# UMEssen/Body-and-Organ-Analysis

Measured on AMD Instinct MI355X. Metric: CT volumes/sec (512^3 @1.5 mm, total+bca) on MI355X, higher is better.
Workload: dtype f16

## Files before the change

body-and-organ-analysis_amd/boa_hip/_lib.py:

```python
from __future__ import annotations

import ctypes as C
import os

_HERE = os.path.dirname(os.path.abspath(__file__))
LIB_PATH = os.environ.get("BOA_HIP_LIB") or os.path.join(_HERE, "libboa_hip.so")

BOA_OK, BOA_EINVAL, BOA_EHIP, BOA_ENOMEM, BOA_EINF = 0, -1, -2, -3, -4
K_CONV_MFMA, K_CONV_FIRST, K_CONVT, K_NORM_FINALIZE, K_HEAD_ACCUM, K_ARGMAX, K_OTHER, K_AGG, K_MORPH, K_RESAMPLE, K_COPY, K_COUNT = range(12)
K_NAMES = ["conv_mfma", "conv_first", "convT_mfma", "norm_finalize", "head_accum", "finalize_argmax", "other", "aggregation",
           "morphology", "resample", "copy_remap"]
CNT_NAMES = ["head_mfma", "head_valu", "conv_ws", "conv_simple", "first_mfma", "first_valu", "f32", "conv_x3", "x3", "head_gather"]
MAX_STAGES = 8


class NetDesc(C.Structure):
    _fields_ = [
        ("n_stages", C.c_int), ("in_channels", C.c_int), ("num_classes", C.c_int),
        ("features", C.c_int * MAX_STAGES), ("kernel", (C.c_int * 3) * MAX_STAGES),
        ("stride", (C.c_int * 3) * MAX_STAGES), ("n_conv_enc", C.c_int * MAX_STAGES),
        ("n_conv_dec", C.c_int * MAX_STAGES), ("patch", C.c_int * 3), ("norm_eps", C.c_float),
        ("lrelu_slope", C.c_float),
    ]

# ... 39 lines not shown
    "boa_finalize_labels": (i32, [vp, vp, vp, i32, ip, vp, i32, i32, i32, vp, i32, vp, ip, ip, vp]),
    "boa_finalize_labels_planes": (i32, [vp, vp, vp, i32, ip, vp, i32, i32, i32, vp, i32, vp, ip, ip, vp, i32, i32]),
    "boa_net_predict_sliding_window_deferred": (i32, [vp, vp, ip, ip, ip, ip, i32, vp, vp, vp, ip, C.POINTER(vp)]),
    "boa_net_apply_deferred": (i32, [vp, vp, vp, vp, vp, ip]),
    "boa_stash_destroy": (None, [vp]),
    "boa_net_create": (i32, [vp, C.POINTER(NetDesc), vp, u64, i32, i32, C.POINTER(vp)]),
    "boa_net_destroy": (None, [vp]),
    "boa_net_weight_count": (u64, [C.POINTER(NetDesc)]),
    "boa_net_load_weights": (i32, [vp, vp, u64]),
    "boa_net_set_mirroring": (i32, [vp, i32]),
    "boa_net_forward": (i32, [vp, vp, ip, ip, i32, vp]),
    "boa_net_predict_sliding_window": (i32, [vp, vp, ip, ip, ip, ip, i32, vp, vp, vp]),
    "boa_net_labels_supported": (i32, [vp, ip, i32]),
    "boa_net_predict_labels_fold": (i32, [vp, vp, ip, ip, ip, ip, i32, vp, vp, i32, i32, vp, i32, vp, ip, ip, vp]),
    "boa_conv_block_test": (i32, [vp, vp, i32, i32, ip, vp, vp, vp, vp, i32, ip, ip, i32, i32, vp]),
    "boa_convtranspose_test": (i32, [vp, vp, i32, i32, ip, vp, vp, i32, ip, vp]),
    "boa_tissue_aggregate": (i32, [vp, vp, vp, vp, vp, vp, i32, i32, i32, vp, vp]),
    "boa_slice_label_presence": (i32, [vp, vp, i32, i32, i32, vp]),
    "boa_tissue_projections": (i32, [vp, vp, vp, i32, i32, i32, vp, i32, vp, vp, vp, vp]),
    "boa_label_hu_histogram": (i32, [vp, vp, vp, vp, u64, i32, i32, vp]),
    "boa_label_hu_mask": (i32, [vp, vp, vp, vp, i32, i32, i32, u64, vp]),
    "boa_group_stats_f64": (i32, [vp, vp, vp, u64, vp, i32, vp, vp]),
    "boa_label_hu_mask_f64": (i32, [vp, vp, vp, vp, i32, C.c_double, C.c_double, u64, vp]),
    "boa_tissue_aggregate_f64": (i32, [vp, vp, vp, vp, vp, vp, i32, i32, i32, vp, vp]),
    "boa_binary_erode": (i32, [vp, vp, vp, vp, i32, i32, i32, i32]),
    "boa_ccl26": (i32, [vp, vp, i32, i32, i32, vp, vp, ip]),
    "boa_ccl_filter_largest": (i32, [vp, vp, vp, u64, vp, i32]),
    "boa_ccl_remove_small": (i32, [vp, vp, vp, u64, C.c_uint32, vp]),
    "boa_ccl_list_components": (i32, [vp, vp, u64, i32, vp, vp, ip]),
    "boa_scatter_u32": (i32, [vp, vp, vp, vp, i32]),
# ... 78 lines not shown
```

body-and-organ-analysis_amd/csrc/conv.h:

```cpp
#pragma once
#include "common.h"

struct ActSrc {
    const __half* data = nullptr;
    const float* ss = nullptr;
    const unsigned* ss16 = nullptr;
    int C = 0;
};

struct ConvGeom {
    int N, Di, Hi, Wi, Do, Ho, Wo;
    int Cout;
    int k[3], s[3];
    int Cin;
};

struct ConvTile {
    int variant;
    int R;
    int w[3];
    int b[3];
    int h[3];
    int xs;
    int tiles[3];
// ... 14 lines not shown
void pack_convt_weights(const float* w , int Cin, int Cout, const int s[3], __half* dst);

int launch_conv_mfma(boa_ctx* ctx, const ActSrc& s0, const ActSrc& s1, const ConvGeom& g, const ConvTile& t,
                     const __half* wpk, const float* bias, float slope, __half* out, float* partials);
int conv_nblk(const ConvTile& t, int cu_count, int Cout);
int conv_ws_nslots(int tiles_per_sample, int cu_count);
int launch_conv_x3(boa_ctx* ctx, const float* src0, const float* ss0, int C0, const float* src1, const float* ss1, int C1,
                   const ConvGeom& g, const ConvTile& t, const __half* wpk, float wscale, const float* bias, float slope, float* out,
                   float* partials);

int launch_norm_finalize(boa_ctx* ctx, float* partials, int nblk, int N, int C, double count,
                         const float* gamma, const float* beta, float eps, float* ss_out, unsigned* ss16_out, int clear);

bool first_mfma_ok(int Cin, const int P[3], const int k[3], int Cout);
bool conv_ws_row_reuse(int R, int k1, int s1, int w1, int b1, int b2);
int convt_mfma_form(int Cin, const int s[3], bool norm_src);
int convt_x3_mt(size_t vin);

int launch_conv_first(boa_ctx* ctx, const float* volume, const int V[3], const int vol_off[3], const int* dev_origins,
                      int N, int Cin, const int P[3], const int k[3], int Cout, const float* w, const float* bias,
                      float* padded_scratch, __half* out, float* partials, int* nblk_out, int flip_mask = 0, float* out32 = nullptr);
int conv_first_nblk(const int P[3], int cu_count);
void conv_first_padded_dims(const int P[3], const int k[3], int out[3]);

int launch_convt_mfma(boa_ctx* ctx, const ActSrc& src, int N, const int din[3], const int s[3], int Cout,
                      const __half* wpk, const float* bias, float slope, __half* out);

int launch_head(boa_ctx* ctx, const __half* act, const float* ss, int F0, const int P[3], int C, const float* w,
                const float* bias, float slope, float* logits_out, const uint16_t* gauss, uint16_t* acc,
                uint16_t* nacc, const int PV[3], const int start[3], size_t plane_stride = 0);
// ... 86 lines not shown
```

body-and-organ-analysis_amd/csrc/conv.hip:

```cpp
#include <stdlib.h>
#include <string.h>

#include <algorithm>
#include <cmath>

#include "conv.h"


size_t conv_wpk_halves(int Cin_total, int Cout, const int k[3]) {
    return (size_t)(Cin_total / 16) * k[0] * k[1] * k[2] * 2 * Cout * 8;
}

void pack_conv_weights(const float* w, int Cin, int Cout, const int k[3], __half* dst) {
    const int taps = k[0] * k[1] * k[2];
    for (int co = 0; co < Cout; ++co)
        for (int ci = 0; ci < Cin; ++ci)
            for (int t = 0; t < taps; ++t) {
                int cc = ci / 16, kh = (ci % 16) / 8, j = ci % 8;
                size_t o = ((((size_t)cc * taps + t) * 2 + kh) * Cout + co) * 8 + j;
                dst[o] = __float2half_rn(w[((size_t)co * Cin + ci) * taps + t]);
            }
}

size_t convt_wpk_halves(int Cin, int Cout, const int s[3]) { return (size_t)s[0] * s[1] * s[2] * Cin * Cout; }
// ... 104 lines not shown
                            if (b0 * b1 * b2 != M) continue;
                            const int b[3] = {b0, b1, b2};
                            int h[3], tl[3];
                            long long HV = 1, covered = 1, tiles = 1;
                            for (int d = 0; d < 3; ++d) {
                                const int ext = b[d] * w[d];
                                h[d] = (ext - 1) * g.s[d] + g.k[d];
                                tl[d] = ceil_div(dims[d], ext);
                                HV *= h[d];
                                covered *= (long long)tl[d] * ext;
                                tiles *= tl[d];
                            }
                            int xs = h[1] * h[2];
                            if (variant == 1 && w0 > 1 && w1 == 1 && w2 >= 8 && w2 <= 16 && g.s[0] == 1 && g.s[2] == 1)
                                while (xs % 16 != w2 % 16) ++xs;
                            if (variant == 1) HV = (long long)h[0] * xs;
                            if (variant == 1 && !conv_ws_supported(g.k, (int)HV)) continue;
                            const size_t lds = variant == 1 ? conv_ws_lds_bytes((int)HV, taps, ncc, g.Cout)
                                                            : conv_lds_bytes((int)HV, taps);
                            if (lds > 160 * 1024 - 2048) continue;
                            const long long nblocks = tiles * (g.Cout / 32) * g.N;
                            const double valid = (double)dims[0] * dims[1] * dims[2];
                            const double waste = (double)covered / valid;
                            const double lds_pen = (g.s[2] > 1 ? 1.25 : 1.0) * (w2 < 16 ? 1.3 : (w2 < 32 ? 1.15 : 1.0));
                            const double t_mfma = (double)taps * R * 32.0 * lds_pen * (x3 ? 2.0 : 1.0);
                            double t_chunk;
                            const double slots = cu_count;
                            if (variant == 1) {
                                const bool res = conv_ws_resident((int)HV, taps, ncc, g.Cout);
                                const double t_prod = (double)h[0] * h[1] * h[2] * 4.3 + (res ? 0.0 : taps * 64.0 / 256.0 * 60.0) + 800.0;
// ... 416 lines not shown
```

body-and-organ-analysis_amd/csrc/conv_ws.hip:

```cpp
#include <stdlib.h>

#include "conv.h"
#include "conv_ws_dev.h"

__global__ __launch_bounds__(64) void k_ws_build_desc(ConvArgs p, int grid, int row, int* __restrict__ out) {
    const int b = (int)blockIdx.x * 64 + (int)threadIdx.x;
    if (b >= grid) return;
    int* r = out + (size_t)b * row * 8;
    int my = 0;
    for (int v = b; v < p.N * p.vw; v += grid) my += p.runs[(v % p.vw) * 8];
    if (my > row - 1) my = row - 1;
    r[0] = my;
    for (int i = 1; i < 8; ++i) r[i] = 0;
    TileSeq s;
    s.n = s.left = s.j = 0;
    for (int k = 0; k < my; ++k) {
        bool new_run = true;
        if (k == 0)
            seq_first_of(p, s, b);
        else
            new_run = seq_next(p, s);
        const TileDesc d = make_desc(p, s, new_run);
        int* e = r + (size_t)(k + 1) * 8;
        e[0] = d.tc.n; e[1] = d.tc.cy; e[2] = d.tc.ox0; e[3] = d.tc.oy0; e[4] = d.tc.oz0; e[5] = d.flags; e[6] = d.vo; e[7] = d.ibase;
// ... 89 lines not shown
            if (jj == 0 || jj == NB - 1)
                __builtin_amdgcn_sched_group_barrier(0x008, 1, 0);
            else if (jj == 1 || jj == NB - 2)
                __builtin_amdgcn_sched_group_barrier(0x008, R >= 2 ? 2 : 1, 0);
            else
                __builtin_amdgcn_sched_group_barrier(0x008, 3, 0);
            (void)cnt;
            if (g + 1 < G) {
                fetch_b(g + 1, jj);
                __builtin_amdgcn_sched_group_barrier(0x100, 1, 0);
            }
        }
    }
}

template <int R, int K0, int K2>
__device__ __forceinline__ void consume_chunk_y_x3(const unsigned char* b0p, const unsigned char* ap, int xs, int h2, int plane, int kh,
                                                   f32x16 (&acc)[R]) {
    constexpr int G = K0 * K2;
    constexpr int NP = G / 2;
    constexpr int NB = R + 2;
    static_assert((G & 1) == 1 && NP >= 1 && R >= 2 && R <= 4, "consume_chunk_y_x3: 3 or 9 groups, 2 .. 4 rows per wave");
    f16x8 ah[2][3], al[2][3];
    f16x8 fh[NB], fl[NB];
    const unsigned char* bhi = b0p - kh * plane;
    auto gtap = [](int g, int dy) { return (((g / K2) * 3 + dy) * K2 + (g % K2)) * 1024; };
    constexpr int GL = G - 1;
    auto fetch_a = [&](int u, int slot) {
        if (u < NP) {
            const int g0 = 2 * u, g1 = g0 + 1;
// ... 89 lines not shown
        for (int r = 0; r < R; ++r) acc[r] = __builtin_amdgcn_mfma_f32_32x32x16_f16(ah[cb][0], fl[r], acc[r], 0, 0, 0);
#pragma unroll
        for (int r = 0; r < R; ++r) acc[r] = __builtin_amdgcn_mfma_f32_32x32x16_f16(al[cb][0], fh[r], acc[r], 0, 0, 0);
#pragma unroll
        for (int r = 0; r < R; ++r) {
            const f16x8& s2 = (r & 1) ? fl[R + r / 2] : fh[R + r / 2];
            acc[r] = __builtin_amdgcn_mfma_f32_32x32x16_f16(ah[cb][2], s2, acc[r], 0, 0, 0);
        }
#pragma unroll
        for (int r = 0; r < R; ++r) {
            const f16x8& s2 = (r & 1) ? fl[R + r / 2] : fh[R + r / 2];
            acc[r] = __builtin_amdgcn_mfma_f32_32x32x16_f16(al[cb][2], s2, acc[r], 0, 0, 0);
        }
    }
}

template <int R, int K0, int K1, int K2, bool YR, bool X3>
__global__ __launch_bounds__(WS_THREADS) void k_conv_ws(ConvArgs p, int total_tiles, int resident_w, int dbg_arg, const int* __restrict__ desc,
                                                        int desc_row) {
#ifdef WS_WITH_TRACE
    const int dbg = dbg_arg;
#else
    constexpr int dbg = 0;
    (void)dbg_arg;
#endif
    extern __shared__ __attribute__((aligned(16))) unsigned char smem[];
    const int tid = threadIdx.x;
    const int lane = tid & 63;
    const int wave = __builtin_amdgcn_readfirstlane(tid >> 6);
    const bool producer = wave >= 4;
    const int l31 = lane & 31;
    const int kh = lane >> 5;
    constexpr int taps = K0 * K1 * K2;
    const int HV = p.h0 * p.xs;
    const int plane = ws_plane_bytes(HV);
    const int ncc = (p.C0 + p.C1) / 16;
    const int wres_bytes = resident_w ? ncc * taps * 1024 : 0;
    const int buf_bytes = resident_w ? 2 * plane : 2 * plane + taps * 1024;
    unsigned char* bufs = smem + wres_bytes;

    const int* __restrict__ drow = desc + (size_t)blockIdx.x * desc_row * 8;
    const int my_tiles = drow[0];
    const int my_chunks = my_tiles * ncc;

    float* const s_bias = (float*)(bufs + 2 * buf_bytes);
    if constexpr (X3) {
        for (int i = tid; i < p.Cout; i += WS_THREADS) s_bias[i] = p.bias[i] * p.wscale;
    }
// ... 75 lines not shown
            if (live && g + 1 < my_chunks) {
                WS_STAMP(1);
                commit(rgA, bufs + ((g + 1) & 1) * buf_bytes);
                if (g + 2 < my_chunks) issue_next(rgA, g + 3 < my_chunks);
                WS_STAMP(3);
            }
            __syncthreads();
        }
        return;
    }

    if (R > 1 && !(dbg & (1024 | 2048))) __builtin_amdgcn_s_setprio(3);
    const int cw = wave & 3;
    int hoff[R];
    {
        const int lz = l31 & (p.w2 - 1);
        const int ly = (l31 >> p.lw2) & (p.w1 - 1);
        const int lx = l31 >> (p.lw2 + p.lw1);
#pragma unroll
        for (int r = 0; r < R; ++r) {
            const int m = cw * R + r;
            const int mz = m & (p.b2 - 1);
            const int my = (m >> p.lb2) & (p.b1 - 1);
            const int mx = m >> (p.lb2 + p.lb1);
            const int tx = mx * p.w0 + lx, ty = my * p.w1 + ly, tz = mz * p.w2 + lz;
            hoff[r] = ((tx * p.s0) * p.xs + (ty * p.s1) * p.h2 + tz * p.s2) * 16 + kh * plane;
        }
    }
    auto vox_rel = [&](int v, int& x, int& y, int& z) {
        x = v >> (p.lw2 + p.lw1);
        y = (v >> p.lw2) & (p.w1 - 1);
        z = v & (p.w2 - 1);
    };
    int srel0;
    {
        int x, y, z;
        vox_rel(l31, x, y, z);
        srel0 = (x * p.Ho + y) * p.Wo + z;
    }
    const size_t out_vox = (size_t)p.Do * p.Ho * p.Wo;
    const int nslots = p.nslots;
    int slot = 0;
    constexpr bool TWO_SETS = (R == 1);
    struct StatSet {
        float s[16], q[16];
    };
    StatSet stA, stB;
#pragma unroll
    for (int i = 0; i < 16; ++i) stA.s[i] = stA.q[i] = stB.s[i] = stB.q[i] = 0.f;
    int st_n = -1, st_cy = 0;
    auto flush_set = [&](StatSet& st, int cy) {
#define WS_HALVE(M, HALF)                                                                                \
    {                                                                                                    \
        const bool up = (l31 & (M)) != 0;                                                                \
        _Pragma("unroll") for (int i = 0; i < (HALF); ++i) {                                             \
            const float ks = up ? st.s[i + (HALF)] : st.s[i], gs = up ? st.s[i] : st.s[i + (HALF)];      \
            const float kq = up ? st.q[i + (HALF)] : st.q[i], gq = up ? st.q[i] : st.q[i + (HALF)];      \
            st.s[i] = ks + __shfl_xor(gs, (M));                                                          \
            st.q[i] = kq + __shfl_xor(gq, (M));                                                          \
        }                                                                                                \
    }
        WS_HALVE(1, 8)
        WS_HALVE(2, 4)
        WS_HALVE(4, 2)
        WS_HALVE(8, 1)
#undef WS_HALVE
        st.s[0] += __shfl_xor(st.s[0], 16);
        st.q[0] += __shfl_xor(st.q[0], 16);
        if (l31 < 16) {
            const int i = ((l31 & 1) << 3) | ((l31 & 2) << 1) | ((l31 & 4) >> 1) | ((l31 & 8) >> 3);
            const int row = cy * 32 + 8 * (i >> 2) + 4 * kh + (i & 3);
            float* pp = p.partials + (((size_t)st_n * p.Cout + row) * 2) * nslots + slot;
            pp[0] = st.s[0];
            pp[nslots] = st.q[0];
        }
#pragma unroll
        for (int i = 0; i < 16; ++i) st.s[i] = st.q[i] = 0.f;
    };
    auto flush_stats = [&]() {
        if (st_n < 0) return;
        if (TWO_SETS && p.cy_fast) {
            flush_set(stA, 0);
            flush_set(stB, 1);
        } else {
            flush_set(stA, st_cy);
        }
    };

    TileDesc cd;
    cd.flags = cd.vo = cd.ibase = 0;
    TileCoord& tc = cd.tc;
    int done_fl = 0, done_vo = 0;
    tc.n = tc.cy = tc.ox0 = tc.oy0 = tc.oz0 = tc.sp = 0;
    if (WS_TRACING && blockIdx.x == 0 && tid == 0) {
        p.trace[WS_TRACE_SLOTS - 4] = __builtin_readcyclecounter();
        p.trace[WS_TRACE_SLOTS - 3] = __builtin_amdgcn_s_memrealtime();
    }
    __syncthreads();
    f32x16 acc[R];
#pragma unroll
    for (int r = 0; r < R; ++r)
#pragma unroll
        for (int i = 0; i < 16; ++i) acc[r][i] = 0.f;
    auto epilogue = [&](const TileCoord& tc, int dfl, int dvo, bool valid) {
        const bool two = TWO_SETS && p.cy_fast;
        if (valid && (tc.n != st_n || (!two && tc.cy != st_cy))) {
            flush_stats();
            st_n = tc.n;
            st_cy = tc.cy;
        }
        const int cout0 = tc.cy * 32;
        const bool full = valid && (dfl & WS_DF_FULL) != 0;
        const size_t ovox = (size_t)(unsigned)dvo;
        const size_t obase = ((size_t)tc.n * p.Cout + cout0) * out_vox + ovox * 16;
        const unsigned olane = ((unsigned)kh * (unsigned)out_vox + (unsigned)srel0) * 32u;
        const unsigned char* const tile_dst = (const unsigned char*)(p.out + obase);
#ifdef WS_TRACE_EPILOGUE
        WS_STAMP(9);
// ... 85 lines not shown
                w[pr * 4 + 2] = cvt_pk_h2(hi4[0], hi4[1]);
                w[pr * 4 + 3] = cvt_pk_h2(hi4[2], hi4[3]);
            }
            if (ok && !(dbg & 4)) {
                WS_GLOBAL unsigned char* dst = sgpr_ptr(tile_dst + (unsigned)mrel * 32u);
                unsigned ol = olane;
                asm volatile("" : "+v"(ol));
                __builtin_nontemporal_store(u32x4_t{w[0], w[1], w[2], w[3]}, (WS_GLOBAL u32x4_t*)(dst + ol));
                __builtin_nontemporal_store(u32x4_t{w[4], w[5], w[6], w[7]}, (WS_GLOBAL u32x4_t*)(dst + ol + 16));
            }
        }
#ifdef WS_TRACE_EPILOGUE
        WS_STAMP(11);
#endif
    };
    f32x16 biasv;
#pragma unroll
    for (int i = 0; i < 16; ++i) biasv[i] = 0.f;
    int bias_cy = -1;
    TileCoord done_tc;
    done_tc.n = done_tc.cy = done_tc.ox0 = done_tc.oy0 = done_tc.oz0 = done_tc.sp = 0;
    for (int k = 0; k < my_tiles + 1; ++k) {
        bool new_run = true;
        const bool more = k < my_tiles;
#ifdef WS_TRACE_EPILOGUE
        WS_STAMP(13);
#endif
        if (more) {
            cd = load_desc(drow, k);
            new_run = (cd.flags & WS_DF_NEWRUN) != 0;
        }
#ifdef WS_TRACE_EPILOGUE
        WS_STAMP(14);
#endif
        if (!(dbg & 8)) epilogue(done_tc, done_fl, done_vo, k > 0);
#pragma unroll
        for (int r = 0; r < R; ++r) asm volatile("" : "=v"(acc[r]));
        if (!more) break;
        if (new_run) {
            flush_stats();
            st_n = -1;
            slot = (int)((unsigned)cd.flags >> 16) * 4 + cw;
        }
        if (!X3 && tc.cy != bias_cy) {
            bias_cy = tc.cy;
            const WS_GLOBAL unsigned char* bbase = sgpr_ptr(p.bias + __builtin_amdgcn_readfirstlane(tc.cy) * 32);
            unsigned bl = (unsigned)kh * 16u;
            asm volatile("" : "+v"(bl));
#pragma unroll
            for (int gq = 0; gq < 4; ++gq) {
                const f32x4_t bv = *(const WS_GLOBAL f32x4_t*)(bbase + bl + 32 * gq);
                biasv[gq * 4 + 0] = bv[0]; biasv[gq * 4 + 1] = bv[1]; biasv[gq * 4 + 2] = bv[2]; biasv[gq * 4 + 3] = bv[3];
            }
            if constexpr (X3) {
#pragma unroll
                for (int i = 0; i < 16; ++i) biasv[i] *= p.wscale;
            }
        }
#ifdef WS_TRACE_EPILOGUE
        WS_STAMP(12);
#endif
        for (int cc = 0; cc < ncc; ++cc) {
            const int g = k * ncc + cc;
            const unsigned char* cur = bufs + (g & 1) * buf_bytes;
            const unsigned char* bp[R];
#pragma unroll
            for (int r = 0; r < R; ++r) {
                int ho = hoff[r];
                asm volatile("" : "+v"(ho));
                bp[r] = cur + ho;
            }
            const unsigned char* ap = (resident_w ? smem + cc * taps * 1024 : cur + 2 * plane) + (X3 ? l31 : kh * 32 + l31) * 16;
            WS_STAMP(4);
            if (dbg & 4096) {
            } else if constexpr (X3) {
                if (cc == 0) {
                    const float* sb = s_bias + tc.cy * 32 + 4 * kh;
#pragma unroll
                    for (int gq = 0; gq < 4; ++gq) {
                        const f32x4_t bv = *(const f32x4_t*)(sb + 8 * gq);
#pragma unroll
                        for (int r = 0; r < R; ++r) {
                            acc[r][gq * 4 + 0] = bv[0]; acc[r][gq * 4 + 1] = bv[1]; acc[r][gq * 4 + 2] = bv[2]; acc[r][gq * 4 + 3] = bv[3];
                        }
                    }
                }
                if constexpr (YR)
                    consume_chunk_y_x3<R, K0, K2>(bp[0], ap, p.xs, p.h2, plane, kh, acc);
                else
                    consume_chunk<R, K0, K1, K2, false, X3>(bp, ap, p.xs, p.h2, acc, biasv);
            } else if constexpr (YR) {
                if (cc == 0)
                    consume_chunk_y<R, K0, K2, true>(bp[0], ap, p.xs, p.h2, acc, biasv);
                else
                    consume_chunk_y<R, K0, K2, false>(bp[0], ap, p.xs, p.h2, acc, biasv);
            } else if (cc == 0)
                consume_chunk<R, K0, K1, K2, true, X3>(bp, ap, p.xs, p.h2, acc, biasv);
            else
                consume_chunk<R, K0, K1, K2, false, X3>(bp, ap, p.xs, p.h2, acc, biasv);
            WS_STAMP(5);
            WS_STAMP(6);
            __syncthreads();
        }
        done_tc.n = __builtin_amdgcn_readfirstlane(tc.n);
        done_tc.cy = __builtin_amdgcn_readfirstlane(tc.cy);
// ... 29 lines not shown
    const bool k333 = k[0] == 3 && k[1] == 3 && k[2] == 3;
    const bool k133 = k[0] == 1 && k[1] == 3 && k[2] == 3;
    return (k333 || k133) && 2 * HV <= WS_PROD * WS_MAXV;
}

template <int R, int K0, int K1, int K2, bool YR, bool X3>
static void launch_ws_y(boa_ctx* ctx, const ConvArgs& a, const ConvTile& t, int total, int grid, int resident, const int* desc, int desc_row) {
    static bool once = (hipFuncSetAttribute((const void*)k_conv_ws<R, K0, K1, K2, YR, X3>, hipFuncAttributeMaxDynamicSharedMemorySize, 160 * 1024), true);
    (void)once;
    hipLaunchKernelGGL((k_conv_ws<R, K0, K1, K2, YR, X3>), dim3(grid), dim3(WS_THREADS), t.lds_bytes + 2048, ctx->stream, a, total, resident,
                       getenv("BOA_WS_DBG") ? atoi(getenv("BOA_WS_DBG")) : 0, desc, desc_row);
}

bool conv_ws_row_reuse(int R, int k1, int s1, int w1, int b1, int b2) {
    return R > 1 && k1 == 3 && s1 == 1 && w1 == 1 && b2 == 1 && b1 % R == 0;
}

template <int R, int K0, int K1, int K2, bool X3>
static void launch_ws_t(boa_ctx* ctx, const ConvArgs& a, const ConvTile& t, int total, int grid, int resident, const int* desc, int desc_row) {
    const bool yr = conv_ws_row_reuse(R, K1, a.s1, a.w1, a.b1, a.b2);
    if (R > 1 && yr)
        launch_ws_y<R, K0, K1, K2, (R > 1), X3>(ctx, a, t, total, grid, resident, desc, desc_row);
    else
        launch_ws_y<R, K0, K1, K2, false, X3>(ctx, a, t, total, grid, resident, desc, desc_row);
}

template <int R, bool X3>
static int launch_ws_r(boa_ctx* ctx, const ConvArgs& a, const ConvTile& t, int total, int grid, int resident, const int* desc, int desc_row) {
    if (a.k0 == 3 && a.k1 == 3 && a.k2 == 3)
        launch_ws_t<R, 3, 3, 3, X3>(ctx, a, t, total, grid, resident, desc, desc_row);
// ... 166 lines not shown
```

body-and-organ-analysis_amd/csrc/net.hip:

```cpp
#include <math.h>
#include <stdlib.h>
#include <string.h>

#include <vector>

#include "conv.h"

namespace {

struct DevBuf {
    void* p = nullptr;
    size_t bytes = 0;
};

enum class NetMode : int { F16 = 0, F32Ref = 1, Split = 2 };

int in_granule(NetMode m) { return m == NetMode::F16 ? 16 : m == NetMode::Split ? 8 : 0; }

struct ActLayout {
    int C;
    int esz;
    bool planar;
    size_t rec() const { return planar ? 32 : (size_t)C * esz; }
    size_t bytes(size_t vox) const { return vox * C * esz; }
// ... 615 lines not shown
    prof.end("convT", U.din, U.Cin, U.Cout, U.s, U.s, 2.0 * f.N * (double)U.din[0] * U.din[1] * U.din[2] * U.s[0] * U.s[1] * U.s[2] * U.Cin * U.Cout,
             nullptr);
    return BOA_OK;
}

static void conv_kernel_info(const boa_net* net, const ConvLayer& L, int info[3]) {
    if (net->mode == NetMode::F32Ref) {
        info[0] = BOA_LK_CONV_F32;
    } else if (L.first) {
        info[0] = first_mfma_ok(net->d.in_channels, net->d.patch, L.g.k, L.g.Cout) ? BOA_LK_FIRST_MFMA : BOA_LK_FIRST_VALU;
    } else {
        const ConvTile& t = L.t;
        info[0] = t.variant == 2 ? BOA_LK_CONV_NS : t.variant == 1 ? BOA_LK_CONV_WS : BOA_LK_CONV_MFMA;
        info[1] = t.R;
        info[2] = t.variant == 1 && conv_ws_row_reuse(t.R, L.g.k[1], L.g.s[1], t.w[1], t.b[1], t.b[2]) ? 1 : 0;
    }
}

static void convt_kernel_info(const boa_net* net, const UpLayer& U, int info[3]) {
    switch (net->mode) {
        case NetMode::F16: {
            const int form = convt_mfma_form(U.Cin, U.s, true);
            info[0] = form == 2 ? BOA_LK_CONVT_DEEP : form == 1 ? BOA_LK_CONVT_RW : BOA_LK_CONVT_MFMA;
            break;
        }
        case NetMode::Split:
            info[0] = BOA_LK_CONVT_X3;
            info[1] = convt_x3_mt((size_t)U.din[0] * U.din[1] * U.din[2]);
            info[2] = (int)std::lround(std::log2((double)U.fold));
            break;
// ... 622 lines not shown
    T_(boa_h2d(ctx, gamma, host_gamma ? host_gamma : ones.data(), Cout * 4));
    T_(boa_h2d(ctx, beta, host_beta ? host_beta : zeros.data(), Cout * 4));
    T_(launch_nchw_to_ndhwc_f16(ctx, dev_in, N, Cin, vin, in16));
    ActSrc a, none;
    a.data = in16; a.ss = nullptr; a.C = Cin;
    T_(launch_conv_mfma(ctx, a, none, g, t, wpk, bias, 0.01f, out16, partials));
    T_(launch_norm_finalize(ctx, partials, nblk, N, Cout, (double)vout, gamma, beta, 1e-5f, ss, nullptr, 1));
    T_(launch_ndhwc_to_nchw_f32(ctx, out16, with_norm_act ? ss : nullptr, 0.01f, N, Cout, vout, dev_out));
    if (rc == BOA_OK) rc = boa_sync(ctx);
#undef T_
    boa_free(ctx, in16); boa_free(ctx, out16); boa_free(ctx, wpk); boa_free(ctx, bias); boa_free(ctx, gamma);
    boa_free(ctx, beta); boa_free(ctx, partials); boa_free(ctx, ss);
    return rc;
}

static int debug_to_nchw(boa_net* net, const ActLayout& lay, const void* tile, const float* ss, float fold, size_t vox, float* out) {
    if (fold == 1.f) return lay.to_nchw(net->ctx, tile, ss, net->d.lrelu_slope, vox, out);
    std::vector<float> tab((size_t)lay.C * 2);
    for (int i = 0; i < lay.C; ++i) {
        tab[2 * i] = 1.f / fold;
        tab[2 * i + 1] = 0.f;
    }
    float* dss = nullptr;
    BOA_TRY(boa_malloc(net->ctx, tab.size() * sizeof(float), (void**)&dss));
    int rc = boa_h2d(net->ctx, dss, tab.data(), tab.size() * sizeof(float));
    if (rc == BOA_OK) rc = lay.to_nchw(net->ctx, tile, dss, 1.f, vox, out);
    if (rc == BOA_OK) rc = boa_sync(net->ctx);
    boa_free(net->ctx, dss);
    return rc;
}
// ... 135 lines not shown
```

include/boa_hip.h:

```cpp
#ifndef BOA_HIP_H
#define BOA_HIP_H

#include <stddef.h>
#include <stdint.h>

#ifdef __cplusplus
extern "C" {
#endif

#define BOA_OK 0
#define BOA_EINVAL (-1)
#define BOA_EHIP (-2)
#define BOA_ENOMEM (-3)
#define BOA_EINF (-4)

typedef struct boa_ctx boa_ctx;
typedef struct boa_net boa_net;

const char* boa_last_error(void);
int boa_version(void);
int boa_init(int device, void* stream, boa_ctx** out);
void boa_destroy(boa_ctx* ctx);
int boa_device_info(boa_ctx* ctx, char* name, int name_len, int* cu_count, size_t* total_mem, size_t* free_mem);
int boa_malloc(boa_ctx* ctx, size_t bytes, void** dev_out);
// ... 89 lines not shown
                                const int* crop_off, const int* crop_dims, int* dev_inf_flag);

typedef struct boa_stash boa_stash;
int boa_net_predict_sliding_window_deferred(boa_net* net, const float* dev_volume, const int V[3], const int PV[3],
                                            const int* vol_off, const int* host_origins, int n_tiles,
                                            const uint16_t* dev_gauss, uint16_t* dev_acc, uint16_t* dev_n,
                                            const int* host_defer_planes, boa_stash** stash_out);
int boa_net_apply_deferred(boa_net* net, const boa_stash* stash, const uint16_t* dev_gauss, uint16_t* dev_acc,
                           uint16_t* dev_n, const int PV[3]);
void boa_stash_destroy(boa_stash* stash);

int boa_conv_block_test(boa_ctx* ctx, const float* dev_in, int N, int Cin, const int dims[3],
                        const float* host_w, const float* host_b, const float* host_gamma, const float* host_beta,
                        int Cout, const int kernel[3], const int stride[3], int with_norm_act, int impl,
                        float* dev_out);
int boa_net_debug_activation(boa_net* net, int kind, int stage, int conv, int tile, float* dev_out, int* channels_out,
                             int dims_out[3]);
#define BOA_LK_FIRST_VALU 1
#define BOA_LK_FIRST_MFMA 2
#define BOA_LK_CONV_WS 3
#define BOA_LK_CONV_NS 4
#define BOA_LK_CONV_MFMA 5
#define BOA_LK_CONV_F32 6
#define BOA_LK_CONVT_X3 7
#define BOA_LK_CONVT_MFMA 8
#define BOA_LK_CONVT_RW 9
#define BOA_LK_CONVT_DEEP 10
#define BOA_LK_CONVT_F32 11
#define BOA_LK_HEAD_X3 12
#define BOA_LK_HEAD_F32 13
// ... 160 lines not shown
```

Before: 0.5869.

## Use 16x16x32 MFMA path for 3x3x3 row-reuse weight-stationary convs

Adds a weight-stationary conv variant for 3x3x3 kernels with row reuse that uses 16x16x32 f16 MFMA instructions instead of the 32x32 form. It comes with a new chunk consumer with explicit scheduling barriers, a reworked stats reduction and an epilogue that uses permlane16 swaps to pack outputs. The tile planner pads xs to a multiple of 16 for these layers. The aim is better MFMA throughput and LDS reuse for the dominant conv layers, at the cost of more accumulator registers and a more complex lane mapping. A conv_block_info query API is also added.

```diff
diff --git a/body-and-organ-analysis_amd/boa_hip/_lib.py b/body-and-organ-analysis_amd/boa_hip/_lib.py
--- a/body-and-organ-analysis_amd/boa_hip/_lib.py
+++ b/body-and-organ-analysis_amd/boa_hip/_lib.py
@@ -77,6 +77,7 @@
     "boa_net_labels_supported": (i32, [vp, ip, i32]),
     "boa_net_predict_labels_fold": (i32, [vp, vp, ip, ip, ip, ip, i32, vp, vp, i32, i32, vp, i32, vp, ip, ip, vp]),
     "boa_conv_block_test": (i32, [vp, vp, i32, i32, ip, vp, vp, vp, vp, i32, ip, ip, i32, i32, vp]),
+    "boa_conv_block_info": (i32, [vp, i32, ip, i32, ip, ip, ip]),
     "boa_convtranspose_test": (i32, [vp, vp, i32, i32, ip, vp, vp, i32, ip, vp]),
     "boa_tissue_aggregate": (i32, [vp, vp, vp, vp, vp, vp, i32, i32, i32, vp, vp]),
     "boa_slice_label_presence": (i32, [vp, vp, i32, i32, i32, vp]),
diff --git a/body-and-organ-analysis_amd/csrc/conv.h b/body-and-organ-analysis_amd/csrc/conv.h
--- a/body-and-organ-analysis_amd/csrc/conv.h
+++ b/body-and-organ-analysis_amd/csrc/conv.h
@@ -52,6 +52,7 @@
 
 bool first_mfma_ok(int Cin, const int P[3], const int k[3], int Cout);
 bool conv_ws_row_reuse(int R, int k1, int s1, int w1, int b1, int b2);
+bool conv_ws_mfma16(int R, const int k[3], int s1, int w1, int b1, int b2, bool x3);
 int convt_mfma_form(int Cin, const int s[3], bool norm_src);
 int convt_x3_mt(size_t vin);
 
diff --git a/body-and-organ-analysis_amd/csrc/conv.hip b/body-and-organ-analysis_amd/csrc/conv.hip
--- a/body-and-organ-analysis_amd/csrc/conv.hip
+++ b/body-and-organ-analysis_amd/csrc/conv.hip
@@ -142,6 +142,8 @@
                             int xs = h[1] * h[2];
                             if (variant == 1 && w0 > 1 && w1 == 1 && w2 >= 8 && w2 <= 16 && g.s[0] == 1 && g.s[2] == 1)
                                 while (xs % 16 != w2 % 16) ++xs;
+                            if (variant == 1 && w2 == 32 && g.s[0] == 1 && g.s[2] == 1 && conv_ws_mfma16(R, g.k, g.s[1], w1, b1, b2, x3))
+                                while (xs % 16 != 0) ++xs;
                             if (variant == 1) HV = (long long)h[0] * xs;
                             if (variant == 1 && !conv_ws_supported(g.k, (int)HV)) continue;
                             const size_t lds = variant == 1 ? conv_ws_lds_bytes((int)HV, taps, ncc, g.Cout)
diff --git a/body-and-organ-analysis_amd/csrc/conv_ws.hip b/body-and-organ-analysis_amd/csrc/conv_ws.hip
--- a/body-and-organ-analysis_amd/csrc/conv_ws.hip
+++ b/body-and-organ-analysis_amd/csrc/conv_ws.hip
@@ -127,6 +127,109 @@
     }
 }
 
+template <int R, bool FIRST>
+__device__ __forceinline__ void consume_chunk_y16(const unsigned char* lds, int b0, int a0, int tp, int vd, int xs, int h2,
+                                                  f32x4_t (&acc)[R][2][2], const f32x4_t (&c0)[2]) {
+    constexpr int NB = R + 2;
+    constexpr int NL = 2 * R;
+    auto ktap = [](int dx, int dy, int dz) { return ((dx * 3 + dy) * 3 + dz) * 1024; };
+    f16x8 a[3][2];
+    f16x8 b[NB][2];
+    f16x8 bl[NL > NB ? NL - NB : 1][2];
+    int p0 = 0, p1 = 0;
+    const int rowb = h2 * 16;
+    auto walk_to = [&](int lane_delta, int off) {
+        p0 = b0 + tp * lane_delta + off;
+        p1 = p0 + vd;
+        asm("" : "+v"(p0), "+v"(p1));
+    };
+    auto read_row = [&](f16x8 (&f)[2]) {
+        f[0] = *(const f16x8*)(lds + p0);
+        f[1] = *(const f16x8*)(lds + p1);
+        p0 += rowb;
+        p1 += rowb;
+        asm("" : "+v"(p0), "+v"(p1));
+    };
+    auto fetch_a = [&](int u, int dy) {
+        const int at = a0 + (u < 3 ? tp * (ktap(0, 0, 1) - ktap(0, 0, 0)) : u == 3 ? tp * (ktap(1, 0, 2) - ktap(0, 0, 2))
+                                   : dy == 0     ? tp * (ktap(2, 1, 2) - ktap(2, 0, 2)) : 0);
+        const int k = u < 3 ? ktap(u, dy, 0) : u == 3 ? ktap(0, dy, 2) : dy == 0 ? ktap(2, 0, 2) : ktap(2, 2, 2);
+#pragma unroll
+        for (int ch = 0; ch < 2; ++ch) a[dy][ch] = *(const f16x8*)(lds + at + k + ch * 256);
+    };
+    auto walk_unit = [&](int u) {
+        if (u < 3)
+            walk_to(16, u * xs * 16);
+        else if (u == 3)
+            walk_to(xs * 16, 2 * 16);
+        else
+            walk_to(rowb, (2 * xs + 2) * 16);
+    };
+    auto mfma4 = [&](const f16x8 (&af)[2], const f16x8 (&bf)[2], int r, bool first) {
+#pragma unroll
+        for (int ch = 0; ch < 2; ++ch)
+#pragma unroll
+            for (int vh = 0; vh < 2; ++vh)
+                acc[r][ch][vh] = __builtin_amdgcn_mfma_f32_16x16x32_f16(af[ch], bf[vh], first ? c0[ch] : acc[r][ch][vh], 0, 0, 0);
+    };
+#pragma unroll
+    for (int dy = 0; dy < 3; ++dy) fetch_a(0, dy);
+    walk_unit(0);
+#pragma unroll
+    for (int jj = 0; jj < NB; ++jj) read_row(b[jj]);
+    __builtin_amdgcn_sched_group_barrier(0x100, 6 + 2 * NB, 0);
+#pragma unroll
+    for (int u = 0; u < 4; ++u) {
+        walk_unit(u + 1);
+#pragma unroll
+        for (int jj = 0; jj < NB; ++jj) {
+#pragma unroll
+            for (int dy = 0; dy < 3; ++dy) {
+                const int r = jj - dy;
+                if (r < 0 || r >= R) continue;
+                mfma4(a[dy], b[jj], r, FIRST && u == 0 && dy == 0);
+            }
+            if (jj == 0 || jj == NB - 1)
+                __builtin_amdgcn_sched_group_barrier(0x008, 4, 0);
+            else if (jj == 1 || jj == NB - 2)
+                __builtin_amdgcn_sched_group_barrier(0x008, 8, 0);
+            else
+                __builtin_amdgcn_sched_group_barrier(0x008, 12, 0);
+            if (u == 3 && jj == R) walk_to(0, (2 * xs + 2 * h2 + 2) * 16);
+            read_row(b[jj]);
+            const int dyf = jj - (R - 1);
+            if (dyf >= 0 && (u < 3 || dyf < 2)) {
+                fetch_a(u + 1, dyf);
+                __builtin_amdgcn_sched_group_barrier(0x100, 4, 0);
+            } else {
+                __builtin_amdgcn_sched_group_barrier(0x100, 2, 0);
+            }
+        }
+    }
+    {
+        const unsigned keep = tp ? 0u : 0xffffffffu;
+#pragma unroll
+        for (int ch = 0; ch < 2; ++ch) {
+            union {
+                f16x8 h;
+                u32x4_t u;
+            } z;
+            z.h = a[1][ch];
+            z.u = z.u & keep;
+            a[1][ch] = z.h;
+        }
+#pragma unroll
+        for (int i = 0; i < NL; ++i) {
+            mfma4(a[i < R ? 0 : 1], i < NB ? b[i] : bl[i < NB ? 0 : i - NB], i < R ? i : i - R, false);
+            __builtin_amdgcn_sched_group_barrier(0x008, 4, 0);
+            if (NB + i < NL) {
+                read_row(bl[i]);
+                __builtin_amdgcn_sched_group_barrier(0x100, 2, 0);
+            }
+        }
+    }
+}
+
 template <int R, int K0, int K2>
 __device__ __forceinline__ void consume_chunk_y_x3(const unsigned char* b0p, const unsigned char* ap, int xs, int h2, int plane, int kh,
                                                    f32x16 (&acc)[R]) {
@@ -246,6 +349,8 @@
         }
     }
 }
+
+__host__ __device__ constexpr bool ws_mfma16(int k0, int k1, int k2, bool yr, bool x3) { return yr && !x3 && k0 == 3 && k1 == 3 && k2 == 3; }
 
 template <int R, int K0, int K1, int K2, bool YR, bool X3>
 __global__ __launch_bounds__(WS_THREADS) void k_conv_ws(ConvArgs p, int total_tiles, int resident_w, int dbg_arg, const int* __restrict__ desc,
@@ -264,6 +369,9 @@
     const int l31 = lane & 31;
     const int kh = lane >> 5;
     constexpr int taps = K0 * K1 * K2;
+    constexpr bool M16 = ws_mfma16(K0, K1, K2, YR, X3);
+    const int n16 = lane & 15;
+    const int q16 = lane >> 4;
     const int HV = p.h0 * p.xs;
     const int plane = ws_plane_bytes(HV);
     const int ncc = (p.C0 + p.C1) / 16;
@@ -369,9 +477,10 @@
     const int cw = wave & 3;
     int hoff[R];
     {
-        const int lz = l31 & (p.w2 - 1);
-        const int ly = (l31 >> p.lw2) & (p.w1 - 1);
-        const int lx = l31 >> (p.lw2 + p.lw1);
+        const int lv = M16 ? n16 : l31;
+        const int lz = lv & (p.w2 - 1);
+        const int ly = (lv >> p.lw2) & (p.w1 - 1);
+        const int lx = lv >> (p.lw2 + p.lw1);
 #pragma unroll
         for (int r = 0; r < R; ++r) {
             const int m = cw * R + r;
@@ -390,19 +499,26 @@
     int srel0;
     {
         int x, y, z;
-        vox_rel(l31, x, y, z);
+        vox_rel(M16 ? 16 * (q16 & 1) + n16 : l31, x, y, z);
         srel0 = (x * p.Ho + y) * p.Wo + z;
+    }
+    int vd16 = 0;
+    if constexpr (M16) {
+        int x, y, z;
+        vox_rel(16, x, y, z);
+        vd16 = ((x * p.s0) * p.xs + (y * p.s1) * p.h2 + z * p.s2) * 16;
     }
     const size_t out_vox = (size_t)p.Do * p.Ho * p.Wo;
     const int nslots = p.nslots;
     int slot = 0;
     constexpr bool TWO_SETS = (R == 1);
+    constexpr int NST = M16 ? 8 : 16;
     struct StatSet {
-        float s[16], q[16];
+        float s[NST], q[NST];
     };
     StatSet stA, stB;
 #pragma unroll
-    for (int i = 0; i < 16; ++i) stA.s[i] = stA.q[i] = stB.s[i] = stB.q[i] = 0.f;
+    for (int i = 0; i < NST; ++i) stA.s[i] = stA.q[i] = stB.s[i] = stB.q[i] = 0.f;
     int st_n = -1, st_cy = 0;
     auto flush_set = [&](StatSet& st, int cy) {
 #define WS_HALVE(M, HALF)                                                                                \
@@ -415,22 +531,37 @@
             st.q[i] = kq + __shfl_xor(gq, (M));                                                          \
         }                                                                                                \
     }
-        WS_HALVE(1, 8)
-        WS_HALVE(2, 4)
-        WS_HALVE(4, 2)
-        WS_HALVE(8, 1)
+        if constexpr (M16) {
+            WS_HALVE(1, 4)
+            WS_HALVE(2, 2)
+            WS_HALVE(4, 1)
+            st.s[0] += __shfl_xor(st.s[0], 8);
+            st.q[0] += __shfl_xor(st.q[0], 8);
+            if (n16 < 8) {
+                const int i = ((n16 & 1) << 2) | (n16 & 2) | ((n16 & 4) >> 2);
+                const int row = cy * 32 + 16 * (i >> 2) + 4 * q16 + (i & 3);
+                float* pp = p.partials + (((size_t)st_n * p.Cout + row) * 2) * nslots + slot;
+                pp[0] = st.s[0];
+                pp[nslots] = st.q[0];
+            }
+        } else {
+            WS_HALVE(1, 8)
+            WS_HALVE(2, 4)
+            WS_HALVE(4, 2)
+            WS_HALVE(8, 1)
+            st.s[0] += __shfl_xor(st.s[0], 16);
+            st.q[0] += __shfl_xor(st.q[0], 16);
+            if (l31 < 16) {
+                const int i = ((l31 & 1) << 3) | ((l31 & 2) << 1) | ((l31 & 4) >> 1) | ((l31 & 8) >> 3);
+                const int row = cy * 32 + 8 * (i >> 2) + 4 * kh + (i & 3);
+                float* pp = p.partials + (((size_t)st_n * p.Cout + row) * 2) * nslots + slot;
+                pp[0] = st.s[0];
+                pp[nslots] = st.q[0];
+            }
+        }
 #undef WS_HALVE
-        st.s[0] += __shfl_xor(st.s[0], 16);
-        st.q[0] += __shfl_xor(st.q[0], 16);
-        if (l31 < 16) {
-            const int i = ((l31 & 1) << 3) | ((l31 & 2) << 1) | ((l31 & 4) >> 1) | ((l31 & 8) >> 3);
-            const int row = cy * 32 + 8 * (i >> 2) + 4 * kh + (i & 3);
-            float* pp = p.partials + (((size_t)st_n * p.Cout + row) * 2) * nslots + slot;
-            pp[0] = st.s[0];
-            pp[nslots] = st.q[0];
-        }
-#pragma unroll
-        for (int i = 0; i < 16; ++i) st.s[i] = st.q[i] = 0.f;
+#pragma unroll
+        for (int i = 0; i < NST; ++i) st.s[i] = st.q[i] = 0.f;
     };
     auto flush_stats = [&]() {
         if (st_n < 0) return;
@@ -452,11 +583,16 @@
         p.trace[WS_TRACE_SLOTS - 3] = __builtin_amdgcn_s_memrealtime();
     }
     __syncthreads();
-    f32x16 acc[R];
-#pragma unroll
-    for (int r = 0; r < R; ++r)
+    f32x16 acc[M16 ? 1 : R];
+#pragma unroll
+    for (int r = 0; r < (M16 ? 1 : R); ++r)
 #pragma unroll
         for (int i = 0; i < 16; ++i) acc[r][i] = 0.f;
+    f32x4_t acc16[M16 ? R : 1][2][2];
+#pragma unroll
+    for (int r = 0; r < (M16 ? R : 1); ++r)
+#pragma unroll
+        for (int i = 0; i < 4; ++i) acc16[r][0][0][i] = acc16[r][0][1][i] = acc16[r][1][0][i] = acc16[r][1][1][i] = 0.f;
     auto epilogue = [&](const TileCoord& tc, int dfl, int dvo, bool valid) {
         const bool two = TWO_SETS && p.cy_fast;
         if (valid && (tc.n != st_n || (!two && tc.cy != st_cy))) {
@@ -572,9 +708,104 @@
         WS_STAMP(11);
 #endif
     };
+    auto epilogue16 = [&](const TileCoord& tc, int dfl, int dvo, bool valid) {
+        if (valid && (tc.n != st_n || tc.cy != st_cy)) {
+            flush_stats();
+            st_n = tc.n;
+            st_cy = tc.cy;
+        }
+        const int cout0 = tc.cy * 32;
+        const bool full = valid && (dfl & WS_DF_FULL) != 0;
+        const size_t ovox = (size_t)(unsigned)dvo;
+        const size_t obase = ((size_t)tc.n * p.Cout + cout0) * out_vox + ovox * 16;
+        const unsigned olane = (unsigned)srel0 * 32u + (unsigned)(q16 >> 1) * 16u;
+        const unsigned char* const tile_dst = (const unsigned char*)(p.out + obase);
+#pragma unroll
+        for (int r = 0; r < R; ++r) {
+            const int m = cw * R + r;
+            const int mx = (m >> (p.lb2 + p.lb1)) * p.w0, my = ((m >> p.lb2) & (p.b1 - 1)) * p.w1, mz = (m & (p.b2 - 1)) * p.w2;
+            const int mrel = (mx * p.Ho + my) * p.Wo + mz;
+            bool ok0 = true, ok1 = true;
+            if (!full) {
+                int x, y, z;
+                vox_rel(n16, x, y, z);
+                ok0 = valid && tc.ox0 + mx + x < p.Do && tc.oy0 + my + y < p.Ho && tc.oz0 + mz + z < p.Wo;
+                vox_rel(16 + n16, x, y, z);
+                ok1 = valid && tc.ox0 + mx + x < p.Do && tc.oy0 + my + y < p.Ho && tc.oz0 + mz + z < p.Wo;
+            }
+            const bool ok = (q16 & 1) ? ok1 : ok0;
+            {
+                StatSet& st = stA;
+                f2_t ps[4], pq[4], pv[2][4];
+#pragma unroll
+                for (int j = 0; j < 4; ++j) {
+                    ps[j] = f2_t{st.s[2 * j], st.s[2 * j + 1]};
+                    pq[j] = f2_t{st.q[2 * j], st.q[2 * j + 1]};
+#pragma unroll
+                    for (int vh = 0; vh < 2; ++vh) pv[vh][j] = f2_t{acc16[r][j >> 1][vh][2 * (j & 1)], acc16[r][j >> 1][vh][2 * (j & 1) + 1]};
+                }
+                if (full) {
+                    asm volatile("; stats16: tile inside the tensor");
+#pragma unroll
+                    for (int vh = 0; vh < 2; ++vh)
+#pragma unroll
+                        for (int j = 0; j < 4; ++j) {
+                            ps[j] += pv[vh][j];
+                            pq[j] = __builtin_elementwise_fma(pv[vh][j], pv[vh][j], pq[j]);
+                        }
+                    asm volatile("" : "+v"(ps[0]), "+v"(ps[1]), "+v"(ps[2]), "+v"(ps[3]), "+v"(pq[0]), "+v"(pq[1]), "+v"(pq[2]), "+v"(pq[3]));
+                } else {
+                    asm volatile("; stats16: tile sticks out");
+#pragma unroll
+                    for (int vh = 0; vh < 2; ++vh) {
+                        const float dm = (vh ? ok1 : ok0) ? 1.f : 0.f;
+                        const f2_t dm2 = f2_t{dm, dm};
+#pragma unroll
+                        for (int j = 0; j < 4; ++j) {
+                            const f2_t vm = pv[vh][j] * dm2;
+                            ps[j] += vm;
+                            pq[j] = __builtin_elementwise_fma(vm, vm, pq[j]);
+                        }
+                    }
+                    asm volatile("" : "+v"(ps[0]), "+v"(ps[1]), "+v"(ps[2]), "+v"(ps[3]), "+v"(pq[0]), "+v"(pq[1]), "+v"(pq[2]), "+v"(pq[3]));
+                }
+#pragma unroll
+                for (int j = 0; j < 4; ++j) {
+                    st.s[2 * j] = ps[j][0]; st.s[2 * j + 1] = ps[j][1];
+                    st.q[2 * j] = pq[j][0]; st.q[2 * j + 1] = pq[j][1];
+                }
+            }
+            __builtin_amdgcn_sched_barrier(0);
+            unsigned w[2][4];
+#pragma unroll
+            for (int ch = 0; ch < 2; ++ch) {
+                float lo4[4], hi4[4];
+#pragma unroll
+                for (int i = 0; i < 4; ++i) {
+                    const auto sw = __builtin_amdgcn_permlane16_swap(__float_as_uint(acc16[r][ch][0][i]), __float_as_uint(acc16[r][ch][1][i]), false, false);
+                    lo4[i] = __uint_as_float(sw[0]);
+                    hi4[i] = __uint_as_float(sw[1]);
+                }
+                w[ch][0] = cvt_pk_h2(lo4[0], lo4[1]);
+                w[ch][1] = cvt_pk_h2(lo4[2], lo4[3]);
+                w[ch][2] = cvt_pk_h2(hi4[0], hi4[1]);
+                w[ch][3] = cvt_pk_h2(hi4[2], hi4[3]);
+            }
+            if (ok) {
+                WS_GLOBAL unsigned char* dst0 = sgpr_ptr(tile_dst + (unsigned)mrel * 32u);
+                WS_GLOBAL unsigned char* dst1 = sgpr_ptr(tile_dst + (unsigned)mrel * 32u + out_vox * 32u);
+                unsigned ol = olane;
+                asm volatile("" : "+v"(ol));
+                __builtin_nontemporal_store(u32x4_t{w[0][0], w[0][1], w[0][2], w[0][3]}, (WS_GLOBAL u32x4_t*)(dst0 + ol));
+                __builtin_nontemporal_store(u32x4_t{w[1][0], w[1][1], w[1][2], w[1][3]}, (WS_GLOBAL u32x4_t*)(dst1 + ol));
+            }
+        }
+    };
     f32x16 biasv;
 #pragma unroll
     for (int i = 0; i < 16; ++i) biasv[i] = 0.f;
+    f32x4_t bias16[2];
+    bias16[0] = bias16[1] = f32x4_t{0.f, 0.f, 0.f, 0.f};
     int bias_cy = -1;
     TileCoord done_tc;
     done_tc.n = done_tc.cy = done_tc.ox0 = done_tc.oy0 = done_tc.oz0 = done_tc.sp = 0;
@@ -591,16 +822,33 @@
 #ifdef WS_TRACE_EPILOGUE
         WS_STAMP(14);
 #endif
-        if (!(dbg & 8)) epilogue(done_tc, done_fl, done_vo, k > 0);
-#pragma unroll
-        for (int r = 0; r < R; ++r) asm volatile("" : "=v"(acc[r]));
+        if constexpr (M16) {
+            if (!(dbg & 8)) epilogue16(done_tc, done_fl, done_vo, k > 0);
+        } else {
+            if (!(dbg & 8)) epilogue(done_tc, done_fl, done_vo, k > 0);
+        }
+        if constexpr (M16) {
+#pragma unroll
+            for (int r = 0; r < R; ++r) asm volatile("" : "=v"(acc16[r][0][0]), "=v"(acc16[r][0][1]), "=v"(acc16[r][1][0]), "=v"(acc16[r][1][1]));
+        } else {
+#pragma unroll
+            for (int r = 0; r < R; ++r) asm volatile("" : "=v"(acc[r]));
+        }
         if (!more) break;
         if (new_run) {
             flush_stats();
             st_n = -1;
             slot = (int)((unsigned)cd.flags >> 16) * 4 + cw;
         }
-        if (!X3 && tc.cy != bias_cy) {
+        if (M16 && tc.cy != bias_cy) {
+            bias_cy = tc.cy;
+            const WS_GLOBAL unsigned char* bbase = sgpr_ptr(p.bias + __builtin_amdgcn_readfirstlane(tc.cy) * 32);
+            unsigned bl = (unsigned)q16 * 16u;
+            asm volatile("" : "+v"(bl));
+#pragma unroll
+            for (int ch = 0; ch < 2; ++ch) bias16[ch] = *(const WS_GLOBAL f32x4_t*)(bbase + bl + 64 * ch);
+        }
+        if (!M16 && !X3 && tc.cy != bias_cy) {
             bias_cy = tc.cy;
             const WS_GLOBAL unsigned char* bbase = sgpr_ptr(p.bias + __builtin_amdgcn_readfirstlane(tc.cy) * 32);
             unsigned bl = (unsigned)kh * 16u;
@@ -628,7 +876,7 @@
                 asm volatile("" : "+v"(ho));
                 bp[r] = cur + ho;
             }
-            const unsigned char* ap = (resident_w ? smem + cc * taps * 1024 : cur + 2 * plane) + (X3 ? l31 : kh * 32 + l31) * 16;
+            const unsigned char* ap = (resident_w ? smem + cc * taps * 1024 : cur + 2 * plane) + (X3 ? l31 : kh * 32 + (M16 ? n16 : l31)) * 16;
             WS_STAMP(4);
             if (dbg & 4096) {
             } else if constexpr (X3) {
@@ -647,6 +895,11 @@
                     consume_chunk_y_x3<R, K0, K2>(bp[0], ap, p.xs, p.h2, plane, kh, acc);
                 else
                     consume_chunk<R, K0, K1, K2, false, X3>(bp, ap, p.xs, p.h2, acc, biasv);
+            } else if constexpr (M16) {
+                if (cc == 0)
+                    consume_chunk_y16<R, true>(smem, (int)(bp[0] - smem), (int)(ap - smem), q16 & 1, vd16, p.xs, p.h2, acc16, bias16);
+                else
+                    consume_chunk_y16<R, false>(smem, (int)(bp[0] - smem), (int)(ap - smem), q16 & 1, vd16, p.xs, p.h2, acc16, bias16);
             } else if constexpr (YR) {
                 if (cc == 0)
                     consume_chunk_y<R, K0, K2, true>(bp[0], ap, p.xs, p.h2, acc, biasv);
@@ -706,6 +959,10 @@
 
 bool conv_ws_row_reuse(int R, int k1, int s1, int w1, int b1, int b2) {
     return R > 1 && k1 == 3 && s1 == 1 && w1 == 1 && b2 == 1 && b1 % R == 0;
+}
+
+bool conv_ws_mfma16(int R, const int k[3], int s1, int w1, int b1, int b2, bool x3) {
+    return ws_mfma16(k[0], k[1], k[2], conv_ws_row_reuse(R, k[1], s1, w1, b1, b2), x3);
 }
 
 template <int R, int K0, int K1, int K2, bool X3>
diff --git a/body-and-organ-analysis_amd/csrc/net.hip b/body-and-organ-analysis_amd/csrc/net.hip
--- a/body-and-organ-analysis_amd/csrc/net.hip
+++ b/body-and-organ-analysis_amd/csrc/net.hip
@@ -653,6 +653,7 @@
         info[0] = t.variant == 2 ? BOA_LK_CONV_NS : t.variant == 1 ? BOA_LK_CONV_WS : BOA_LK_CONV_MFMA;
         info[1] = t.R;
         info[2] = t.variant == 1 && conv_ws_row_reuse(t.R, L.g.k[1], L.g.s[1], t.w[1], t.b[1], t.b[2]) ? 1 : 0;
+        if (t.variant == 1 && conv_ws_mfma16(t.R, L.g.k, L.g.s[1], t.w[1], t.b[1], t.b[2], net->mode == NetMode::Split)) info[2] = 2;
     }
 }
 
@@ -1305,6 +1306,26 @@
     return rc;
 }
 
+extern "C" int boa_conv_block_info(boa_ctx* ctx, int Cin, const int dims[3], int Cout, const int kernel[3], const int stride[3], int info[3]) {
+    BOA_REQUIRE(ctx && dims && kernel && stride && info, "conv info: NULL argument");
+    ConvGeom g;
+    g.N = TILE_REF_BATCH; g.Di = dims[0]; g.Hi = dims[1]; g.Wi = dims[2]; g.Cout = Cout; g.Cin = Cin;
+    for (int a = 0; a < 3; ++a) {
+        g.k[a] = kernel[a];
+        g.s[a] = stride[a];
+    }
+    g.Do = (dims[0] + 2 * ((kernel[0] - 1) / 2) - kernel[0]) / stride[0] + 1;
+    g.Ho = (dims[1] + 2 * ((kernel[1] - 1) / 2) - kernel[1]) / stride[1] + 1;
+    g.Wo = (dims[2] + 2 * ((kernel[2] - 1) / 2) - kernel[2]) / stride[2] + 1;
+    ConvTile t;
+    BOA_REQUIRE(choose_conv_tile(g, ctx->cu_count, &t), "conv info: no tile configuration");
+    info[0] = t.variant == 2 ? BOA_LK_CONV_NS : t.variant == 1 ? BOA_LK_CONV_WS : BOA_LK_CONV_MFMA;
+    info[1] = t.R;
+    info[2] = t.variant != 1 ? 0 : conv_ws_mfma16(t.R, g.k, g.s[1], t.w[1], t.b[1], t.b[2], false) ? 2
+              : conv_ws_row_reuse(t.R, g.k[1], g.s[1], t.w[1], t.b[1], t.b[2])                        ? 1 : 0;
+    return BOA_OK;
+}
+
 static int debug_to_nchw(boa_net* net, const ActLayout& lay, const void* tile, const float* ss, float fold, size_t vox, float* out) {
     if (fold == 1.f) return lay.to_nchw(net->ctx, tile, ss, net->d.lrelu_slope, vox, out);
     std::vector<float> tab((size_t)lay.C * 2);
diff --git a/include/boa_hip.h b/include/boa_hip.h
--- a/include/boa_hip.h
+++ b/include/boa_hip.h
@@ -127,6 +127,7 @@
                         const float* host_w, const float* host_b, const float* host_gamma, const float* host_beta,
                         int Cout, const int kernel[3], const int stride[3], int with_norm_act, int impl,
                         float* dev_out);
+int boa_conv_block_info(boa_ctx* ctx, int Cin, const int dims[3], int Cout, const int kernel[3], const int stride[3], int info[3]);
 int boa_net_debug_activation(boa_net* net, int kind, int stage, int conv, int tile, float* dev_out, int* channels_out,
                              int dims_out[3]);
 #define BOA_LK_FIRST_VALU 1
```

New measurement: 0.5820. Within noise of the previous version (-0.8%).
